# ebeauce/Seismic_BPMF

Hardware: AMD Instinct MI355X
Metric: million network-CC-samples/s (matched filter) (higher is better)
Workload: dtype f32

## Files before the change

### include/bpmf_hip.h

```cpp
#ifndef BPMF_HIP_H
#define BPMF_HIP_H

#include <stddef.h>
#include <stdint.h>

#ifdef __cplusplus
extern "C" {
#endif

typedef void *bpmf_stream_t;


const char *bpmf_last_error(void);

int bpmf_device_count(void);

int bpmf_device_info(int device, char *name, size_t name_len, size_t *total_mem_bytes,
                     int *compute_units);

#define BPMF_KERNEL_MF_MAIN 0
#define BPMF_KERNEL_BP_BEAM 1
#define BPMF_KERNEL_COUNT 2
void bpmf_profile_enable(int enable);
int bpmf_profile_count(int which_kernel);
int bpmf_profile_get_ms(int which_kernel, int launch_index, float *milliseconds);
int bpmf_profile_get_device(int which_kernel, int launch_index);

int bpmf_release_device_memory(int device);
int bpmf_device_memory_held(int device, size_t *device_bytes, size_t *pinned_bytes);
int bpmf_host_call_stats(double *out, int n);

int bpmf_set_option(const char *name, long value);
int bpmf_get_option(const char *name, long *value, long *default_value);


#define BPMF_MF_DATA_PREPARED 1
#define BPMF_MF_FORCE_DIRECT 2

size_t bpmf_mf_workspace_bytes(size_t L, size_t N, size_t T, size_t S, size_t C);

int bpmf_mf_prepare_data_dev(const float *d_data, size_t L, size_t N, size_t S, size_t C,
                             void *d_workspace, size_t workspace_bytes, bpmf_stream_t stream);

int bpmf_mf_run_dev(const float *d_templates, const int32_t *d_moveouts,
                    const float *d_weights, const float *d_data, size_t step, size_t L,
                    size_t N, size_t T, size_t S, size_t C, size_t n_corr, int network_sum,
                    int flags, void *d_workspace, size_t workspace_bytes,
                    bpmf_stream_t stream, float *d_cc_out);

#define BPMF_MF_LAUNCH_INFO_FIELDS 13
int bpmf_mf_launch_info(size_t step, size_t L, size_t N, size_t T, size_t S, size_t C, size_t n_corr,
                        int network_sum, int flags, int64_t *out);

int bpmf_mf_run(const float *templates, const int32_t *moveouts, const float *weights,
                const float *data, size_t step, size_t L, size_t N, size_t T, size_t S,
                size_t C, size_t n_corr, int network_sum, int flags, int device,
                float *cc_out);

int bpmf_mf_run_multi(const float *templates, const int32_t *moveouts, const float *weights,
                      const float *data, size_t step, size_t L, size_t N, size_t T, size_t S,
                      size_t C, size_t n_corr, int network_sum, int flags, int n_devices,
                      const int *devices, float *cc_out);

int bpmf_mf_shard_bounds(const float *weights, size_t T, size_t S, size_t C, size_t n_blocks,
                         size_t *bounds_out);

#define BPMF_BP_STRICT 0
#define BPMF_BP_FLEXIBLE 1
#define BPMF_BP_REDUCE_MAX 0
#define BPMF_BP_REDUCE_NONE 1

typedef struct bpmf_bp_plan bpmf_bp_plan;

int bpmf_bp_plan_create(const int32_t *moveouts, const float *w_sources, size_t K, size_t S,
                        size_t P, int device, int32_t source_id_offset, bpmf_bp_plan **plan);
void bpmf_bp_plan_destroy(bpmf_bp_plan *plan);

typedef struct {
    int32_t n_groups;
    int32_t tile;
    int32_t lds_bytes;
    int32_t gather_bytes;
    int32_t stations_max;
    int32_t waves_per_cu;
    int32_t n_classes;
    int32_t class_tile[3], class_sources[3], class_groups[3], class_stations_max[3];
} bpmf_bp_plan_stats;
int bpmf_bp_plan_info(const bpmf_bp_plan *plan, bpmf_bp_plan_stats *out);

size_t bpmf_bp_workspace_bytes(const bpmf_bp_plan *plan, size_t N, size_t C);

int bpmf_bp_run_dev(const bpmf_bp_plan *plan, const float *d_features,
                    const float *d_w_phases, size_t N, size_t C, int out_of_bounds,
                    int reduce, void *d_workspace, size_t workspace_bytes,
                    bpmf_stream_t stream, float *d_beam_out, int32_t *d_arg_out);

int bpmf_bp_run(const float *features, const int32_t *moveouts, const float *w_phases,
                const float *w_sources, size_t N, size_t K, size_t S, size_t C, size_t P,
                int out_of_bounds, int reduce, int device, float *beam_out, int32_t *arg_out);

int bpmf_bp_run_multi(const float *features, const int32_t *moveouts, const float *w_phases,
                      const float *w_sources, size_t N, size_t K, size_t S, size_t C, size_t P,
                      int out_of_bounds, int reduce, int n_devices, const int *devices,
// ... 142 lines not shown
```

### seismic_bpmf_amd/_lib.py

```python
import ctypes as C
import os

_HERE = os.path.dirname(os.path.abspath(__file__))
LIBPATH = os.path.join(_HERE, "lib", "libbpmf_hip.so")

_f = C.POINTER(C.c_float)
_i = C.POINTER(C.c_int32)
_u64 = C.POINTER(C.c_uint64)
_sz = C.c_size_t
_vp = C.c_void_p

class BpPlanStats(C.Structure):
    _fields_ = ([(n, C.c_int32) for n in ("n_groups", "tile", "lds_bytes", "gather_bytes",
                                          "stations_max", "waves_per_cu", "n_classes")] +
                [(n, C.c_int32 * 3) for n in ("class_tile", "class_sources", "class_groups",
                                              "class_stations_max")])


SIGNATURES = {
    "bpmf_last_error": (C.c_char_p, []),
    "bpmf_device_count": (C.c_int, []),
    "bpmf_device_info": (C.c_int, [C.c_int, C.c_char_p, _sz, C.POINTER(_sz), C.POINTER(C.c_int)]),
    "bpmf_set_option": (C.c_int, [C.c_char_p, C.c_long]),
    "bpmf_get_option": (C.c_int, [C.c_char_p, C.POINTER(C.c_long), C.POINTER(C.c_long)]),
# ... 102 lines not shown
    if rc != 0:
        msg = lib().bpmf_last_error().decode("utf-8", "replace")
        raise BpmfHipError(f"{what} failed (status {rc}): {msg}")


def last_error():
    return lib().bpmf_last_error().decode("utf-8", "replace")


def host_call_stats():
    buf = (C.c_double * 11)()
    k = lib().bpmf_host_call_stats(buf, 11)
    names = ("total_ms", "first_kernel_start_ms", "host_copy_ms", "device_wait_ms", "pieces", "fill_threads",
             "pinned_wait_ms", "copy_enqueue_ms", "plan_ms", "reserve_ms", "stragglers")
    out = {n: float(buf[i]) for i, n in enumerate(names[:k])}
    for n in ("pieces", "fill_threads", "stragglers"):
        if n in out:
            out[n] = int(out[n])
    return out


def device_count():
    n = lib().bpmf_device_count()
    if n < 0:
        check(n, "bpmf_device_count")
    return n


def device_info(device=0):
    name = C.create_string_buffer(256)
    mem = _sz(0)
    cus = C.c_int(0)
    check(lib().bpmf_device_info(device, name, 256, C.byref(mem), C.byref(cus)), "bpmf_device_info")
    return {"name": name.value.decode(), "total_mem_bytes": mem.value, "compute_units": cus.value}


KERNEL_MF_MAIN, KERNEL_BP_BEAM = 0, 1


def set_option(name, value):
    check(lib().bpmf_set_option(name.encode(), int(value)), f"bpmf_set_option({name})")


def get_option(name):
    val, dflt = C.c_long(0), C.c_long(0)
    check(lib().bpmf_get_option(name.encode(), C.byref(val), C.byref(dflt)), f"bpmf_get_option({name})")
    return val.value, dflt.value


MF_FAMILIES = ("direct", "workgroup", "wave", "split16")
MF_REFUSALS = (None, "grid too large", "more than 65535 templates on the generic kernel")


def mf_launch_info(step, L, N, T, n_stations, n_components, network_sum=True, flags=0):
    out = (C.c_int64 * 13)()
    check(lib().bpmf_mf_launch_info(step, L, N, T, n_stations, n_components, (N - L) // step + 1, 1 if network_sum else 0, int(flags), out),
          "bpmf_mf_launch_info")
    names = ("family", "maxr", "maxt", "ntile", "fused", "csplit", "sqrt_norm", "step1", "prologue", "lags_per_wg",
             "lds_bytes", "grid", "refusal")
    info = dict(zip(names, (int(x) for x in out)))
    for n in ("fused", "csplit", "sqrt_norm", "step1", "prologue"):
        info[n] = bool(info[n])
    info["family"] = MF_FAMILIES[info["family"]]
    info["refusal"] = MF_REFUSALS[info["refusal"]]
    return info


class options:

    def __init__(self, **kv):
        self.kv = {k.replace("__", "."): v for k, v in kv.items()}

    def __enter__(self):
        self.old = {k: get_option(k)[0] for k in self.kv}
        for k, v in self.kv.items():
            set_option(k, v)
        return self

    def __exit__(self, *exc):
        for k, v in self.old.items():
            set_option(k, v)
        return False


def release_device_memory(device=-1):
    check(lib().bpmf_release_device_memory(int(device)), "bpmf_release_device_memory")


def device_memory_held(device=-1):
    dv, pn = _sz(0), _sz(0)
    check(lib().bpmf_device_memory_held(int(device), C.byref(dv), C.byref(pn)), "bpmf_device_memory_held")
    return dv.value, pn.value


def profile_enable(on=True):
    lib().bpmf_profile_enable(1 if on else 0)


def _closed_launches(which):
    out = []
    for i in range(lib().bpmf_profile_count(which)):
        ms = C.c_float(0.0)
        if lib().bpmf_profile_get_ms(which, i, C.byref(ms)) == 0:
            out.append((i, ms.value))
    return out


def profile_devices(which):
    return [lib().bpmf_profile_get_device(which, i) for i, _ in _closed_launches(which)]


def profile_times_ms(which):
    return [ms for _, ms in _closed_launches(which)]


COMPAT_SWITCHES = ("mf.compat_exclusive_last_lag", "mf.compat_sqrt_norm", "mf.compat_range_all_channels",
                   "mf.compat_sequential_csum", "bp.compat_first_computed", "bp.compat_strict_upper_only",
# ... 30 lines not shown
```

### seismic_bpmf_amd/csrc/common.h

```cpp
#pragma once
#include <hip/hip_runtime.h>
#include <cstdarg>
#include <cstdint>
#include <cstdio>

namespace bpmf {

char* last_error_buf();
void set_error(const char* fmt, ...);

constexpr int CSUM_CHUNK = 1024;
constexpr float MAX_NORM = 1000.0f;

void profile_mark(int which, int edge, hipStream_t stream);

inline size_t align_up(size_t x, size_t a) { return (x + a - 1) / a * a; }

enum Option {
    OPT_BP_LDS_KB, OPT_BP_MAX_GROUP, OPT_BP_TPT, OPT_BP_REORDER, OPT_BP_DUAL,
    OPT_BP_FAST, OPT_BP_FAST_UNIFORM, OPT_BP_SPLIT, OPT_BP_VERBOSE, OPT_BP_FAST_TILE, OPT_BP_HALVES, OPT_BP_DIRECT, OPT_MF_WAVE_KERNEL, OPT_MF_MAX_MFMA_STEP, OPT_MF_HOST_BATCH_KB,
    OPT_MF_HOST_PIECE_KB, OPT_MF_VERBOSE, OPT_MF_TILES_PER_WAVE, OPT_MF_BOUNDARY_PRIO, OPT_MF_FUSED_PROLOGUE, OPT_DEBUG_POISON_OUTPUT,
    OPT_DEBUG_VIRTUAL_DEVICES, OPT_MULTI_PEER_FANOUT, OPT_MF_HOST_PIECE_LAGS, OPT_BP_HOST_PIECE_SAMPLES,
    OPT_HOST_CACHE_LIMIT_MB, OPT_BP_SLOT_PRIO, OPT_MF_CHANNEL_SPLIT, OPT_STATS_BUCKETED_MEDIAN, OPT_STATS_ROW_GRID_MIN_N, OPT_STATS_KURT_FULL_CHUNKS, OPT_MF_SPLIT16, OPT_DEBUG_FAIL_PEER_COPY,
    OPT_DEBUG_COPY_STALL_MS,
    OPT_MF_COMPAT_EXCLUSIVE_LAST_LAG, OPT_MF_COMPAT_SQRT_NORM, OPT_BP_COMPAT_FIRST_COMPUTED,
    OPT_MF_COMPAT_RANGE_ALL_CHANNELS, OPT_MF_COMPAT_SEQUENTIAL_CSUM, OPT_BP_COMPAT_STRICT_UPPER_ONLY,
    OPT_BP_COMPAT_RANGE_ALL_STATIONS, OPT_COUNT
};
long option(Option which);
unsigned long long option_generation();

hipError_t device_counts(int* n_logical, int* n_physical);
int physical_device(int logical);
extern thread_local int t_logical_device;

class DeviceGuard {
public:
    explicit DeviceGuard(int device) : DeviceGuard(device, physical_device(device)) {}
    DeviceGuard(int logical, int physical)
    {
        prev_logical_ = t_logical_device;
        t_logical_device = logical;
        err_ = hipGetDevice(&prev_);
        if (err_ == hipSuccess && prev_ != physical) {
            err_ = hipSetDevice(physical);
            switched_ = err_ == hipSuccess;
        }
    }
    ~DeviceGuard()
    {
        if (switched_) (void)hipSetDevice(prev_);
        t_logical_device = prev_logical_;
    }
    DeviceGuard(const DeviceGuard&) = delete;
    DeviceGuard& operator=(const DeviceGuard&) = delete;
    hipError_t error() const { return err_; }
private:
    int prev_ = 0, prev_logical_ = -1;
    bool switched_ = false;
    hipError_t err_ = hipSuccess;
};

}

#define BPMF_HIP_CHECK(expr)                                                          \
    do {                                                                              \
        hipError_t _e = (expr);                                                       \
        if (_e != hipSuccess) {                                                       \
            bpmf::set_error("%s failed: %s (%s:%d)", #expr, hipGetErrorString(_e),    \
                            __FILE__, __LINE__);                                      \
            return -2;                                                                \
        }                                                                             \
    } while (0)

#define BPMF_LAUNCH_CHECK() BPMF_HIP_CHECK(hipGetLastError())

#define BPMF_BIND_DEVICE(device)                 \
// ... 3 lines not shown
```

### seismic_bpmf_amd/csrc/mf.hip

```cpp
#include "common.h"
#include "context.h"
#include "mf_split_api.h"
#include <system_error>
#include <thread>
#include <chrono>
#include <vector>
#include <mutex>
#include <utility>
#include <cstring>
#include <algorithm>
#include "../../include/bpmf_hip.h"

#include <cstdlib>

namespace bpmf {

typedef float f32x16 __attribute__((ext_vector_type(16)));


__device__ __forceinline__ int2 mf_lag_range(bool any, long long mv_min, long long mv_max, long long step,
                                             long long L, long long N, long long n_corr, int exclusive_last)
{
    int2 r = make_int2(1, 0);
    if (any && N >= L) {
// ... 201 lines not shown
__device__ __forceinline__ int mf_pad(int x) { return x + (x >> 4); }

__host__ __device__ inline int mf_kpad(int L) { return (L + 15 + 15) / 16 * 16; }
__host__ __device__ inline int mf_band_len(int L) { return mf_kpad(L) + 16; }
__host__ __device__ inline int mf_window_len(int L) { return MF_LAGS_PER_WG - 16 + mf_kpad(L); }
__host__ __device__ inline int mf_buf_floats(int L)
{
    const int W = mf_window_len(L);
    return mf_band_len(L) + (W + (W >> 4) + 1);
}
__host__ inline size_t mf_lds_bytes(int L) { return ((size_t)2 * mf_buf_floats(L) + 64) * sizeof(float); }

__device__ __forceinline__ bool mf_tile_of_block(unsigned bid, int T, int n_lag_blocks, int& t,
                                                 long long& lag_block)
{
    const unsigned xcd = bid & 7u, i = bid >> 3;
    const unsigned total = (unsigned)n_lag_blocks * (unsigned)T;
    const unsigned per_xcd = (total + 7u) >> 3;
    const unsigned flat = xcd * per_xcd + i;
    t = (int)(flat % (unsigned)T);
    lag_block = (long long)(flat / (unsigned)T);
    return i < per_xcd && flat < total;
}

template <int NR, int STRIDE>
__device__ __forceinline__ void mf_stage_rows(float (&rd)[NR], __amdgpu_buffer_rsrc_t rs,
                                              long long first, int idx)
{
    const unsigned o = (unsigned)((first + idx) * 4);
    if (first >= 0) {
#pragma unroll
        for (int r = 0; r < NR; ++r)
            rd[r] = __builtin_bit_cast(float, __builtin_amdgcn_raw_buffer_load_b32(rs, (int)(o + STRIDE * 4u * r), 0, 0));
    } else {
        unsigned oo = o;
#pragma unroll
        for (int r = 0; r < NR; ++r) {
            asm volatile("" : "+v"(oo));
            rd[r] = __builtin_bit_cast(float, __builtin_amdgcn_raw_buffer_load_b32(rs, (int)oo, 0, 0));
            oo += STRIDE * 4u;
        }
    }
}
template <int NR, int STRIDE>
__device__ __forceinline__ void mf_stage_band(float (&rt)[NR], __amdgpu_buffer_rsrc_t rs, int idx)
{
    int o0 = (idx - 15) * 4;
    asm volatile("" : "+v"(o0));
    rt[0] = __builtin_bit_cast(float, __builtin_amdgcn_raw_buffer_load_b32(rs, o0, 0, 0));
#pragma unroll
    for (int r = 1; r < NR; ++r)
        rt[r] = __builtin_bit_cast(float, __builtin_amdgcn_raw_buffer_load_b32(
                                              rs, idx * 4 + (STRIDE * r - 15) * 4, 0, 0));
}

template <bool NETWORK_SUM, int MAXR, int MAXT, bool STEP1, bool SQRT_NORM = false>
__global__ __launch_bounds__(MF_THREADS, 2) void mf_mfma_kernel(
    const float* __restrict__ tmpl, const int4* __restrict__ chan_rec,
    const float* __restrict__ data, const float* __restrict__ e_d,
    const int2* __restrict__ range, int L, long long N, int T, int n_ch, long long n_corr, int step,
    float* __restrict__ out, int n_lag_blocks, int prio, int lag_block0)
{
    extern __shared__ float smem[];
    const int Kpad = mf_kpad(L);
    const int tp_len = mf_band_len(L);
    const int W = mf_window_len(L);
    const int buf_floats = mf_buf_floats(L);

    const int tid = threadIdx.x;
    const int lane = tid & 63;
    const int wv = tid >> 6;
    const int a = lane & 15;
    const int kq = lane >> 4;

    int t;
    long long lag_block;
    if (!mf_tile_of_block(blockIdx.x, T, n_lag_blocks, t, lag_block)) return;
    lag_block += lag_block0;
    const long long lag0 = lag_block * MF_LAGS_PER_WG;
    const int2 rgi = range[t];
    const int2 rg = make_int2(rgi.x * step, rgi.y * step);
    const long long nwin = N - L + 1;

    f32x4 sum[4];
#pragma unroll
    for (int u = 0; u < 4; ++u) sum[u] = (f32x4){0.0f, 0.0f, 0.0f, 0.0f};

    const bool wg_valid = rg.x <= rg.y && !(lag0 > rg.y || lag0 + MF_LAGS_PER_WG - 1 < rg.x);
    const bool wg_inside = lag0 >= rg.x && lag0 + MF_LAGS_PER_WG - 1 <= rg.y;
    const long long lag_w = lag0 + (long long)wv * MF_LAGS_PER_WAVE + 16 * a + 4 * kq;

    if (wg_valid) {
        const int a_base = 15 - a + kq;
        const int b_base = 1088 * wv + 17 * a + kq;
        const int4* __restrict__ recs = chan_rec + (size_t)t * (n_ch + 2);

        float rd[MAXR], rt[MAXT];
        auto issue_stage = [&](int ch, int mvc) {
            const __amdgpu_buffer_rsrc_t rs_d = __builtin_amdgcn_make_buffer_rsrc(
                (void*)(data + (size_t)ch * (size_t)N), 0, (int)(N * 4), 0x00020000);
            mf_stage_rows<MAXR, MF_THREADS>(rd, rs_d, lag0 + mvc, tid);
            const __amdgpu_buffer_rsrc_t rs_t = __builtin_amdgcn_make_buffer_rsrc(
                (void*)(tmpl + ((size_t)t * n_ch + ch) * (size_t)L), 0, L * 4, 0x00020000);
            mf_stage_band<MAXT, MF_THREADS>(rt, rs_t, tid);
        };
        auto write_stage = [&](float* tp, float* dw) {
// ... 455 lines not shown
                    float cc = 0.0f;
                    if (ok) {
                        cc = mf_cc_of<SQRT_NORM>(acc[u][r], et, ed[u][r]);
                        if (!NETWORK_SUM)
                            out[((size_t)t * n_corr + (STEP1 ? lag : (long long)((unsigned)lag / (unsigned)step))) * n_ch + ch] = cc;
                    }
                    if (NETWORK_SUM) sum[u][r] = __fmaf_rn(w, cc, sum[u][r]);
                }
            }
            }
            rec = rec1;
            rec1 = rec2;
            ri += REC_STRIDE;
            MF_PHASE(3);
#ifdef BPMF_PHASE_CYCLES
            ++ph_n_;
#endif
        }
    }
    if constexpr (CSPLIT) {
        __syncthreads();
        const long long lag = lag0 + tid;
        float s = 0.0f;
        if (wave_valid) {
            for (int i = 0; i < n_used; ++i) s = __fmaf_rn(__int_as_float(l_rec[i].z), exch[i * 256 + tid], s);
        }
        if (lag < n_corr) out[(size_t)t * n_corr + lag] = s;
    } else if (NETWORK_SUM) {
#pragma unroll
        for (int u = 0; u < NTILE; ++u) {
            const long long lag = lag_w + 256 * u;
            float* dst = out + (size_t)t * n_corr + lag;
            if (STEP1 && lag + 3 < n_corr) {
                *(f32x4u*)dst = sum[u];
            } else {
#pragma unroll
                for (int r = 0; r < 4; ++r) {
                    const unsigned smp = (unsigned)(lag + r);
                    const long long i = STEP1 ? (long long)smp : (long long)(smp / (unsigned)step);
                    if ((STEP1 || smp % (unsigned)step == 0) && i < n_corr) out[(size_t)t * n_corr + i] = sum[u][r];
                }
            }
        }
    }
#ifdef BPMF_PHASE_CYCLES
    if (lane == 0 && ph_n_) {
        for (int i = 0; i < 4; ++i) atomicAdd(&g_mf_phase[i], ph_acc_[i]);
        atomicAdd(&g_mf_phase[4], (unsigned long long)ph_n_);
        atomicAdd(&g_mf_phase[5], 1ull);
    }
#endif
}

template <bool NETWORK_SUM, bool SQRT_NORM = false>
__global__ __launch_bounds__(256) void mf_direct_kernel(
    const float* __restrict__ tmpl, const int* __restrict__ mv, const float* __restrict__ wgt,
    const float* __restrict__ data, const float* __restrict__ e_t,
    const float* __restrict__ e_d, const int2* __restrict__ range, long long step, int L,
    long long N, int n_ch, long long n_corr, float* __restrict__ out,
    const double* __restrict__ cs_local = nullptr, const double* __restrict__ cs_off = nullptr, long long nq = 0)
{
    const long long i = (long long)blockIdx.x * blockDim.x + threadIdx.x;
    const int t = blockIdx.y;
    if (i >= n_corr) return;
    const int2 rg = range[t];
    const bool ok = i >= rg.x && i <= rg.y;
    const long long nwin = N - L + 1;
    float sum = 0.0f;
    if (ok) {
        for (int ch = 0; ch < n_ch; ++ch) {
            const float w = wgt[(size_t)t * n_ch + ch];
            if (w == 0.0f) continue;
            const long long j = i * step + mv[(size_t)t * n_ch + ch];
            const float* tp = tmpl + ((size_t)t * n_ch + ch) * (size_t)L;
            const float* d = data + (size_t)ch * (size_t)N + j;
            float num = 0.0f;
            for (int l = 0; l < L; ++l) num = __fmaf_rn(tp[l], d[l], num);
            float cc = 0.0f;
            if constexpr (SQRT_NORM) {
                float et = 0.0f;
                for (int l = 0; l < L; ++l) et = __fmaf_rn(tp[l], tp[l], et);
                const double* lo = cs_local + (size_t)ch * (size_t)N;
                const double* of = cs_off + (size_t)ch * (size_t)nq;
                const long long nh = j + L - 1;
                const double hi = of[nh / CSUM_CHUNK] + lo[nh];
                const double low = j > 0 ? of[(j - 1) / CSUM_CHUNK] + lo[j - 1] : 0.0;
                const float den2 = et * (float)(hi - low);
                if (den2 > 1.0e-6f) cc = num / sqrtf(den2);
            } else {
                const float nrm = e_t[(size_t)t * n_ch + ch] * e_d[(size_t)ch * nwin + j];
                if (nrm < MAX_NORM) cc = num * nrm;
            }
            if (NETWORK_SUM)
                sum = __fmaf_rn(w, cc, sum);
            else
                out[((size_t)t * n_corr + i) * n_ch + ch] = cc;
        }
    }
    if (NETWORK_SUM) out[(size_t)t * n_corr + i] = sum;
}

struct MfWorkspace {
    double* local;
    double* tot;
    double* off;
    float* e_d;
// ... 37 lines not shown
                  L, T, S, C);
        return -1;
    }
    if (N < L) {
        set_error("matched filter: data (N=%zu) shorter than the templates (L=%zu)", N, L);
        return -1;
    }
    if (n_corr != (N - L) / step + 1) {
        set_error("matched filter: n_corr=%zu but (N-L)/step+1=%zu", n_corr, (N - L) / step + 1);
        return -1;
    }
    if (N > 0x7fffffffull || T * S * C > 0x7fffffffull || L > 0x7fffffffull) {
        set_error("matched filter: dimension exceeds the int32 index range");
        return -1;
    }
    return 0;
}

struct MfLaunch {
    long long off_lo = 0, off_hi = -1;
    bool first_piece = true;
};

static std::mutex g_split_days_mutex;
struct SplitDay { const void* data; size_t N, n_ch; };
static std::vector<std::pair<const void*, SplitDay>> g_split_days;
static void split_day_note(const void* ws_base, const void* data, size_t N, size_t n_ch, bool with_split)
{
    std::lock_guard<std::mutex> g(g_split_days_mutex);
    for (size_t i = 0; i < g_split_days.size(); ++i)
        if (g_split_days[i].first == ws_base) { g_split_days.erase(g_split_days.begin() + i); break; }
    if (with_split) {
        if (g_split_days.size() >= 64) g_split_days.erase(g_split_days.begin());
        g_split_days.push_back({ws_base, {data, N, n_ch}});
    }
}
static bool split_day_known(const void* ws_base, const void* data, size_t N, size_t n_ch)
{
    std::lock_guard<std::mutex> g(g_split_days_mutex);
    for (auto& e : g_split_days)
        if (e.first == ws_base) return e.second.data == data && e.second.N == N && e.second.n_ch == n_ch;
    return false;
}

enum MfFamily { MF_DIRECT = 0, MF_WORKGROUP = 1, MF_WAVE = 2, MF_SPLIT16 = 3 };
enum MfRefusal { MF_ACCEPTED = 0, MF_GRID_TOO_LARGE = 1, MF_TOO_MANY_TEMPLATES = 2 };
static const char* const MF_REFUSAL_TEXT[] = {"", "grid too large", "generic kernel supports at most 65535 templates per call"};

struct MfVariant {
    int family, refusal;
    int maxr, maxt;
    int ntile;
    bool fused, csplit;
    bool sqrt_norm, step1, prologue;
    size_t lags_wg, lds, grid;
};

constexpr int MF_WAVE_MAXT = 5;
constexpr int mf_wave_maxr(int ntile) { return ntile == 4 ? 20 : (ntile == 2 ? 12 : 8); }
static size_t mf_grid(size_t T, size_t n_blocks) { return 8 * ((T * n_blocks + 7) / 8); }

static MfVariant mf_choose(size_t step, size_t L, size_t N, size_t T, size_t n_ch, size_t n_corr, int network_sum,
                           int flags, bool ranged)
{
    MfVariant v = {};
    v.sqrt_norm = option(OPT_MF_COMPAT_SQRT_NORM) != 0;
    v.step1 = step == 1;
    v.prologue = true;
    const size_t n_offsets = (n_corr - 1) * step + 1;
    const size_t n_lag_blocks = (n_offsets + MF_LAGS_PER_WG - 1) / MF_LAGS_PER_WG;
    const int need_r = (mf_window_len((int)L) + MF_THREADS - 1) / MF_THREADS;
    const int need_t = (mf_band_len((int)L) + MF_THREADS - 1) / MF_THREADS;
    const bool mfma = step <= (size_t)option(OPT_MF_MAX_MFMA_STEP) && !(flags & BPMF_MF_FORCE_DIRECT) && need_r <= 24 &&
                      need_t <= 9 && T * (n_lag_blocks + 8) < 0x7fffffffull && N < ((size_t)1 << 30) - 8192;
    if (!mfma) {
        v.family = MF_DIRECT;
        v.lags_wg = 256;
        v.grid = (n_corr + 255) / 256 * T;
        if (T > 65535) v.refusal = MF_TOO_MANY_TEMPLATES;
        return v;
    }
    constexpr size_t SP_MIN_BLOCKS = 128;
    const size_t sp_blocks = (n_offsets + sp::LAGS_PER_WG - 1) / sp::LAGS_PER_WG;
    const bool sp_small = option(OPT_MF_SPLIT16) == 1 && T * sp_blocks < SP_MIN_BLOCKS;
    if (option(OPT_MF_SPLIT16) != 0 && sp::usable(L, N) && !sp_small) {
        v.family = MF_SPLIT16;
        v.lags_wg = sp::LAGS_PER_WG;
        v.grid = mf_grid(T, sp_blocks);
        return v;
    }
    if (option(OPT_MF_WAVE_KERNEL) == 0 || mf_kpad((int)L) > 272) {
        v.family = MF_WORKGROUP;
        v.maxr = need_r <= 20 && need_t <= 5 ? 20 : 24;
        v.maxt = v.maxr == 20 ? 5 : 9;
        v.lags_wg = MF_LAGS_PER_WG;
        v.lds = mf_lds_bytes((int)L);
        v.grid = mf_grid(T, n_lag_blocks);
        return v;
    }
    v.family = MF_WAVE;
    const size_t waves4 = T * n_lag_blocks * 4;
    v.ntile = waves4 >= 8192 ? 4 : (waves4 >= 1024 ? 2 : 1);
    const long forced = option(OPT_MF_TILES_PER_WAVE);
    if (forced == 1 || forced == 2 || forced == 4) v.ntile = (int)forced;
    v.maxr = mf_wave_maxr(v.ntile);
    v.maxt = MF_WAVE_MAXT;
    v.fused = v.ntile < 4 && n_ch <= 256 && option(OPT_MF_FUSED_PROLOGUE) != 0;
    v.prologue = !v.fused;
    const long csplit_max = option(OPT_MF_CHANNEL_SPLIT);
    v.csplit = v.ntile == 1 && v.fused && network_sum && v.step1 && n_ch <= 32 && !ranged && csplit_max > 0 &&
               waves4 * 4 <= (size_t)csplit_max;
    v.lags_wg = v.csplit ? (size_t)256 : (size_t)4 * 256 * v.ntile;
    const size_t n_blocks_w = (n_offsets + v.lags_wg - 1) / v.lags_wg;
    if (T * (n_blocks_w + 8) >= 0x7fffffffull) v.refusal = MF_GRID_TOO_LARGE;
    v.grid = mf_grid(T, n_blocks_w);
    const int Wbuf = v.ntile < 4 ? 64 * v.maxr : 256 * v.ntile - 16 + mf_kpad((int)L);
    v.lds = (size_t)4 * (mf_band_len((int)L) + (Wbuf + 2 * (Wbuf >> 4) + 2 + 63) / 64 * 64 + 64) * sizeof(float) + 256 +
            (v.fused ? 64 + (n_ch + MF_REC_TERMINATORS) * sizeof(int4) : 0) +
            (v.csplit ? n_ch * 256 * sizeof(float) : 0);
    return v;
}

}

using namespace bpmf;

extern "C" size_t bpmf_mf_workspace_bytes(size_t L, size_t N, size_t T, size_t S, size_t C)
{
    return mf_carve(nullptr, L, N, T, S * C).bytes;
}

static int mf_prepare_range(const float* d_data, size_t L, size_t N, size_t n_ch, const MfWorkspace& ws,
                            hipStream_t stream, size_t samp_lo, size_t samp_hi)
{
    const size_t nq = (N + CSUM_CHUNK - 1) / CSUM_CHUNK;
    const size_t nwin = N - L + 1;
    const size_t q_lo = samp_lo / CSUM_CHUNK, q_hi = (samp_hi + CSUM_CHUNK - 1) / CSUM_CHUNK;
    if (q_hi <= q_lo) return 0;
    {
        size_t n = n_ch * (q_hi - q_lo);
        mf_csum_local_kernel<<<dim3((unsigned)((n + 63) / 64)), dim3(64), 0, stream>>>(
            d_data, n_ch, N, nq, ws.local, ws.tot, q_lo, q_hi - q_lo);
        BPMF_LAUNCH_CHECK();
    }
    mf_csum_offsets_kernel<<<dim3((unsigned)((n_ch + 63) / 64)), dim3(64), 0, stream>>>(
        ws.tot, n_ch, nq, ws.off, q_lo, q_hi);
    BPMF_LAUNCH_CHECK();
    const size_t w_lo = samp_lo >= L - 1 ? samp_lo - (L - 1) : 0;
    const size_t w_hi = samp_hi >= N ? nwin : (samp_hi >= L - 1 ? std::min(nwin, samp_hi - (L - 1)) : 0);
    if (w_hi > w_lo) {
        mf_window_energy_kernel<<<dim3((unsigned)((w_hi - w_lo + 255) / 256), (unsigned)n_ch), dim3(256), 0,
                                  stream>>>(ws.local, ws.off, n_ch, N, nq, L, nwin,
                                            option(OPT_MF_COMPAT_SQRT_NORM) != 0 ? 1 : 0, ws.e_d, w_lo, w_hi);
        BPMF_LAUNCH_CHECK();
    }
    return 0;
}

extern "C" int bpmf_mf_prepare_data_dev(const float* d_data, size_t L, size_t N, size_t S, size_t C,
                                        void* d_workspace, size_t workspace_bytes,
                                        bpmf_stream_t stream_)
{
    hipStream_t stream = (hipStream_t)stream_;
    const size_t n_ch = S * C;
// ... 66 lines not shown
        set_error("bpmf_mf_run_dev: internal error: a range of lag blocks under mf.split16");
        return -1;
    }
    const size_t n_offsets = (n_corr - 1) * step + 1;
    const size_t off_lo = ranged ? (size_t)lc.off_lo : 0;
    const size_t off_hi = ranged ? std::min<size_t>((size_t)lc.off_hi, n_offsets) : n_offsets;
    if (off_hi <= off_lo) return 0;
    if (v.family == MF_SPLIT16 && !split_day_known(d_workspace, d_data, N, n_ch)) {
        set_error("bpmf_mf_run_dev: option mf.split16 is on but the day in this workspace was prepared without it (or is "
                  "another day): call bpmf_mf_prepare_data_dev again, or drop BPMF_MF_DATA_PREPARED");
        return -1;
    }
    if (v.refusal) {
        set_error("bpmf_mf_run_dev: %s", MF_REFUSAL_TEXT[v.refusal]);
        return -1;
    }
    const int exclusive_last = (option(OPT_MF_COMPAT_EXCLUSIVE_LAST_LAG) != 0 ? 1 : 0) |
                               (option(OPT_MF_COMPAT_RANGE_ALL_CHANNELS) != 0 ? 2 : 0);
    if (v.prologue) {
        mf_prologue_kernel<<<dim3((unsigned)T), dim3(64), 0, stream>>>(
            d_templates, d_moveouts, d_weights, (int)T, (int)n_ch, (long long)step, (long long)L, (long long)N,
            (long long)n_corr, exclusive_last, v.sqrt_norm ? 1 : 0, ws.e_t, ws.range, ws.chan_rec);
        BPMF_LAUNCH_CHECK();
    }
    if (lc.first_piece && !network_sum)
        BPMF_HIP_CHECK(hipMemsetAsync(d_cc_out, 0, T * n_corr * n_ch * sizeof(float), stream));
    else if (lc.first_piece && option(OPT_DEBUG_POISON_OUTPUT) != 0)
        BPMF_HIP_CHECK(hipMemsetAsync(d_cc_out, 0xFF, T * n_corr * sizeof(float), stream));

    const size_t nb_lo = off_lo / v.lags_wg, nb_cnt = (off_hi - off_lo + v.lags_wg - 1) / v.lags_wg;
    const dim3 grid((unsigned)mf_grid(T, nb_cnt));
    const int prio = (int)option(OPT_MF_BOUNDARY_PRIO);
    profile_mark(BPMF_KERNEL_MF_MAIN, 0, stream);
    const int rc = with_sum_step_norm(network_sum != 0, v.step1, v.sqrt_norm, [&](auto ns_c, auto s1_c, auto sq_c) -> int {
        constexpr bool NS = decltype(ns_c)::value, S1 = decltype(s1_c)::value, SQ = decltype(sq_c)::value;
        auto workgroup = [&](auto maxr_c, auto maxt_c) -> int {
            auto kern = mf_mfma_kernel<NS, decltype(maxr_c)::value, decltype(maxt_c)::value, S1, SQ>;
            if (v.lds > 64 * 1024)
                BPMF_HIP_CHECK(hipFuncSetAttribute((const void*)kern, hipFuncAttributeMaxDynamicSharedMemorySize, 160 * 1024));
            kern<<<grid, dim3(MF_THREADS), v.lds, stream>>>(
                d_templates, ws.chan_rec, d_data, ws.e_d, ws.range, (int)L, (long long)N, (int)T, (int)n_ch,
                (long long)n_corr, (int)step, d_cc_out, (int)nb_cnt, prio, (int)nb_lo);
            return 0;
        };
        auto wave = [&](auto ntile_c, auto fused_c, auto csplit_c) -> int {
            constexpr int NTILE = decltype(ntile_c)::value;
            mf_mfma_wave_kernel<NS, mf_wave_maxr(NTILE), MF_WAVE_MAXT, S1, NTILE, SQ, decltype(fused_c)::value,
                                decltype(csplit_c)::value><<<grid, dim3(MF_THREADS), v.lds, stream>>>(
                d_templates, ws.chan_rec, d_data, ws.e_d, ws.range, (int)L, (long long)N, (int)T, (int)n_ch,
                (long long)n_corr, (int)step, d_cc_out, (int)nb_cnt, prio, d_moveouts, d_weights, exclusive_last,
                (int)nb_lo);
            return 0;
        };
        auto direct = [&]() -> int {
            mf_direct_kernel<NS, SQ><<<dim3((unsigned)((n_corr + 255) / 256), (unsigned)T), dim3(256), 0, stream>>>(
                d_templates, d_moveouts, d_weights, d_data, ws.e_t, ws.e_d, ws.range, (long long)step, (int)L,
                (long long)N, (int)n_ch, (long long)n_corr, d_cc_out, ws.local, ws.off,
                (long long)((N + CSUM_CHUNK - 1) / CSUM_CHUNK));
            return 0;
        };
        const std::true_type yes{};
        const std::false_type no{};
        switch (v.family) {
            case MF_SPLIT16:
                return sp::run(d_templates, d_moveouts, ws.sp_day, ws.sp_batch, ws.chan_rec, ws.e_d, ws.range, step, L, N,
                               T, n_ch, n_corr, network_sum, v.sqrt_norm ? 1 : 0, 0, nb_cnt, d_cc_out, stream);
            case MF_WORKGROUP:
                return v.maxr == 20 ? workgroup(IntC<20>{}, IntC<5>{})
                                    : workgroup(IntC<24>{}, IntC<9>{});
            case MF_WAVE:
                if constexpr (NS && S1)
                    if (v.csplit) return wave(IntC<1>{}, yes, yes);
                if (v.ntile == 4) return wave(IntC<4>{}, no, no);
                if (v.ntile == 2) return v.fused ? wave(IntC<2>{}, yes, no) : wave(IntC<2>{}, no, no);
                return v.fused ? wave(IntC<1>{}, yes, no) : wave(IntC<1>{}, no, no);
            default:
                return direct();
        }
    });
    if (rc) return rc;
    BPMF_LAUNCH_CHECK();
    profile_mark(BPMF_KERNEL_MF_MAIN, 1, stream);
    return 0;
}

}

extern "C" int bpmf_mf_run_dev(const float* d_templates, const int32_t* d_moveouts, const float* d_weights,
                               const float* d_data, size_t step, size_t L, size_t N, size_t T, size_t S, size_t C,
                               size_t n_corr, int network_sum, int flags, void* d_workspace, size_t workspace_bytes,
                               bpmf_stream_t stream, float* d_cc_out)
{
    if (!d_templates || !d_moveouts || !d_weights || !d_data || !d_workspace || !d_cc_out) {
        set_error("bpmf_mf_run_dev: null pointer");
        return -1;
    }
    return mf_run_dev(d_templates, d_moveouts, d_weights, d_data, step, L, N, T, S, C, n_corr, network_sum, flags,
                      d_workspace, workspace_bytes, (hipStream_t)stream, d_cc_out, MfLaunch());
}

extern "C" int bpmf_mf_launch_info(size_t step, size_t L, size_t N, size_t T, size_t S, size_t C, size_t n_corr,
                                   int network_sum, int flags, int64_t* out)
{
    if (!out) {
        set_error("bpmf_mf_launch_info: null pointer");
        return -1;
    }
    if (int rc = mf_check_sizes(step, L, N, T, S, C, n_corr)) return rc;
    const MfVariant v = mf_choose(step, L, N, T, S * C, n_corr, network_sum, flags, false);
    const int64_t fields[BPMF_MF_LAUNCH_INFO_FIELDS] = {
        v.family, v.maxr, v.maxt, v.ntile, v.fused, v.csplit, v.sqrt_norm, v.step1, v.prologue,
        (int64_t)v.lags_wg, (int64_t)v.lds, (int64_t)v.grid, v.refusal};
    memcpy(out, fields, sizeof(fields));
    return 0;
}


static std::vector<size_t> mf_batch_starts(size_t T, size_t TB)
{
    std::vector<size_t> taper;
    size_t a = 2, b2 = 3, used = 0;
    while (a < TB && used + a <= T) {
        taper.push_back(a);
        used += a;
        const size_t next = b2;
        b2 = a + b2;
        a = next;
    }
    const size_t rest = T - used;
    const size_t n_full = (rest + TB - 1) / TB;
    std::vector<size_t> bt(1, 0);
    for (size_t i = 0; i < n_full; ++i)
        bt.push_back(bt.back() + rest / n_full + (i < rest % n_full ? 1 : 0));
    for (size_t i = taper.size(); i-- > 0;) bt.push_back(bt.back() + taper[i]);
    return bt;
}

static int bpmf_mf_run_impl(const float* templates, const int32_t* moveouts, const float* weights,
                           const float* data, size_t step, size_t L, size_t N, size_t T, size_t S,
                           size_t C, size_t n_corr, int network_sum, int flags, int device,
                           float* cc_out)
{
    if (!templates || !moveouts || !weights || !data || !cc_out) {
        set_error("bpmf_mf_run: null pointer");
        return -1;
    }
    if (int rc = mf_check_sizes(step, L, N, T, S, C, n_corr)) return rc;
    BPMF_BIND_DEVICE(device);
    t_call_stats = HostCallStats();
    const double t_call0 = host_now_ms();
    const size_t n_ch = S * C;
    const size_t row_bytes = n_corr * (network_sum ? 1 : n_ch) * sizeof(float);
    const long e_b = option(OPT_MF_HOST_BATCH_KB), e_p = option(OPT_MF_HOST_PIECE_KB);
    const size_t batch_bytes = e_b > 0 ? (size_t)e_b << 10 : (size_t)1 << 30;
    const size_t PIECE = e_p > 0 ? (size_t)e_p << 10 : (size_t)64 << 20;
    size_t TB = std::max<size_t>(1, batch_bytes / std::max<size_t>(row_bytes, 1));
    if (!e_b) TB = std::max<size_t>(TB, 8);
    TB = std::min(T, TB);
    const std::vector<size_t> bt = mf_batch_starts(T, TB);
    const size_t n_batch = bt.size() - 1;
    const size_t b_tp = T * n_ch * L * sizeof(float), b_mv = T * n_ch * sizeof(int32_t),
                 b_w = T * n_ch * sizeof(float), b_d = n_ch * N * sizeof(float),
                 b_out = TB * row_bytes, b_ws = bpmf_mf_workspace_bytes(L, N, TB, S, C);
    DeviceContext* ctx = device_context(device);
    if (!ctx) return -2;
// ... 180 lines not shown
```

### seismic_bpmf_amd/csrc/util.hip

```cpp
#include "common.h"
#include "../../include/bpmf_hip.h"

#include <atomic>
#include <cstring>
#include <mutex>
#include <vector>

namespace bpmf {

char* last_error_buf()
{
    static thread_local char buf[512] = {0};
    return buf;
}

void set_error(const char* fmt, ...)
{
    va_list ap;
    va_start(ap, fmt);
    vsnprintf(last_error_buf(), 512, fmt, ap);
    va_end(ap);
}

}

namespace bpmf {
namespace {
struct OptionDef { const char* name; long dflt; long lo, hi; bool plan; };
const OptionDef OPTION_DEFS[OPT_COUNT] = {
    {"bp.lds_kb", 80, 8, 160, true},
    {"bp.max_group", 4096, 1, 1 << 20, true},
    {"bp.tpt", 2, 1, 2, true},
    {"bp.reorder", 1, 0, 1, true},
    {"bp.dual", 1, 0, 1, true},
    {"bp.fast", 1, 0, 1, true},
    {"bp.fast_uniform", 1, 0, 1, true},
    {"bp.split", -1, -1, 1 << 16, false},
    {"bp.verbose", 0, 0, 1, false},
    {"bp.fast_tile", 0, 0, 512, true},
    {"bp.halves", 1, 0, 1, true},
    {"bp.direct", 0, 0, 1, true},
    {"mf.wave_kernel", 1, 0, 1, false},
    {"mf.max_mfma_step", 64, 0, 1 << 20, false},
    {"mf.host_batch_kb", 0, 0, 1L << 30, false},
    {"mf.host_piece_kb", 0, 0, 1L << 30, false},
    {"mf.verbose", 0, 0, 1, false},
    {"mf.tiles_per_wave", 0, 0, 4, false},
    {"mf.boundary_prio", 1, 0, 3, false},
    {"mf.fused_prologue", 1, 0, 1, false},
    {"debug.poison_output", 0, 0, 1, false},
    {"debug.virtual_devices", 0, 0, 64, false},
    {"multi.peer_fanout", 1, 0, 1, false},
    {"mf.host_piece_lags", 131072, 0, 1 << 24, false},
    {"bp.host_piece_samples", 131072, 0, 1 << 24, false},
    {"host.cache_limit_mb", 0, 0, 1L << 30, false},
    {"bp.slot_prio", 1, 0, 2, false},
    {"mf.channel_split", 2048, 0, 1 << 24, false},
    {"stats.bucketed_median", 2, 0, 2, false},
    {"stats.row_grid_min_n", 131072, -1, 1 << 30, false},
    {"stats.kurt_full_chunks", 1, 0, 1, false},
    {"mf.split16", 0, 0, 2, false},
    {"debug.fail_peer_copy", 0, 0, 1, false},
    {"debug.copy_stall_ms", 0, 0, 2000, false},
    {"mf.compat_exclusive_last_lag", 0, 0, 1, false},
    {"mf.compat_sqrt_norm", 0, 0, 1, false},
    {"bp.compat_first_computed", 0, 0, 1, false},
    {"mf.compat_range_all_channels", 0, 0, 1, false},
    {"mf.compat_sequential_csum", 0, 0, 1, false},
    {"bp.compat_strict_upper_only", 0, 0, 1, true},
    {"bp.compat_range_all_stations", 0, 0, 1, true},
};
std::atomic<long> g_options[OPT_COUNT];
std::once_flag g_options_once;
void init_options()
{
    for (int i = 0; i < OPT_COUNT; ++i) g_options[i].store(OPTION_DEFS[i].dflt, std::memory_order_relaxed);
}
int find_option(const char* name)
{
    if (!name) return -1;
    for (int i = 0; i < OPT_COUNT; ++i)
        if (strcmp(name, OPTION_DEFS[i].name) == 0) return i;
    return -1;
}
}

std::atomic<unsigned long long> g_option_generation{0};
unsigned long long option_generation() { return g_option_generation.load(std::memory_order_relaxed); }

long option(Option which)
{
    std::call_once(g_options_once, init_options);
    return g_options[which].load(std::memory_order_relaxed);
}

thread_local int t_logical_device = -1;

hipError_t device_counts(int* n_logical, int* n_physical)
{
    int n = 0;
    const hipError_t e = hipGetDeviceCount(&n);
    if (e != hipSuccess) n = 0;
    const long v = option(OPT_DEBUG_VIRTUAL_DEVICES);
    if (n_physical) *n_physical = n;
    if (n_logical) *n_logical = (v > 0 && n > 0) ? (int)v : n;
    return e;
}

int physical_device(int logical)
{
    if (logical < 0 || option(OPT_DEBUG_VIRTUAL_DEVICES) <= 0) return logical;
    int n = 0;
    if (hipGetDeviceCount(&n) != hipSuccess || n < 1) return logical;
    return logical % n;
}
}
// ... 185 lines not shown
```

Measured before the change: 4357.

## Add hand-scheduled chained MFMA wave kernel for 4-tile network-sum matched filter

Adds a new wave-level matched-filter kernel for the 4-tile, step-1, network-sum case with template length up to 256. It processes channels as a chain, issuing the next channel's global loads mid-way through the current one, and interleaves LDS reads with MFMA issue using explicit waitcnt and sched_barrier placement. The aim is to hide load and LDS latency and cut per-channel stalls. The new option mf.chain_tiles defaults to on, so eligible shapes route to this kernel, at the cost of heavy inline-asm scheduling that is fragile and specific to one template-padding size.

```diff
diff --git a/include/bpmf_hip.h b/include/bpmf_hip.h
--- a/include/bpmf_hip.h
+++ b/include/bpmf_hip.h
@@ -48,7 +48,7 @@
                     int flags, void *d_workspace, size_t workspace_bytes,
                     bpmf_stream_t stream, float *d_cc_out);
 
-#define BPMF_MF_LAUNCH_INFO_FIELDS 13
+#define BPMF_MF_LAUNCH_INFO_FIELDS 14
 int bpmf_mf_launch_info(size_t step, size_t L, size_t N, size_t T, size_t S, size_t C, size_t n_corr,
                         int network_sum, int flags, int64_t *out);
 
diff --git a/seismic_bpmf_amd/_lib.py b/seismic_bpmf_amd/_lib.py
--- a/seismic_bpmf_amd/_lib.py
+++ b/seismic_bpmf_amd/_lib.py
@@ -178,8 +178,8 @@
 MF_REFUSALS = (None, "grid too large", "more than 65535 templates on the generic kernel")
 
 
-def mf_launch_info(step, L, N, T, n_stations, n_components, network_sum=True, flags=0):
-    out = (C.c_int64 * 13)()
+def mf_launch_info(step, L, N, T, n_stations, n_components, network_sum=True, flags=0, detail=False):
+    out = (C.c_int64 * 14)()
     check(lib().bpmf_mf_launch_info(step, L, N, T, n_stations, n_components, (N - L) // step + 1, 1 if network_sum else 0, int(flags), out),
           "bpmf_mf_launch_info")
     names = ("family", "maxr", "maxt", "ntile", "fused", "csplit", "sqrt_norm", "step1", "prologue", "lags_per_wg",
@@ -189,6 +189,8 @@
         info[n] = bool(info[n])
     info["family"] = MF_FAMILIES[info["family"]]
     info["refusal"] = MF_REFUSALS[info["refusal"]]
+    if detail:
+        info["chain_tiles"] = int(out[13])
     return info
 
 
diff --git a/seismic_bpmf_amd/csrc/common.h b/seismic_bpmf_amd/csrc/common.h
--- a/seismic_bpmf_amd/csrc/common.h
+++ b/seismic_bpmf_amd/csrc/common.h
@@ -22,7 +22,7 @@
     OPT_MF_HOST_PIECE_KB, OPT_MF_VERBOSE, OPT_MF_TILES_PER_WAVE, OPT_MF_BOUNDARY_PRIO, OPT_MF_FUSED_PROLOGUE, OPT_DEBUG_POISON_OUTPUT,
     OPT_DEBUG_VIRTUAL_DEVICES, OPT_MULTI_PEER_FANOUT, OPT_MF_HOST_PIECE_LAGS, OPT_BP_HOST_PIECE_SAMPLES,
     OPT_HOST_CACHE_LIMIT_MB, OPT_BP_SLOT_PRIO, OPT_MF_CHANNEL_SPLIT, OPT_STATS_BUCKETED_MEDIAN, OPT_STATS_ROW_GRID_MIN_N, OPT_STATS_KURT_FULL_CHUNKS, OPT_MF_SPLIT16, OPT_DEBUG_FAIL_PEER_COPY,
-    OPT_DEBUG_COPY_STALL_MS,
+    OPT_DEBUG_COPY_STALL_MS, OPT_MF_CHAIN_TILES,
     OPT_MF_COMPAT_EXCLUSIVE_LAST_LAG, OPT_MF_COMPAT_SQRT_NORM, OPT_BP_COMPAT_FIRST_COMPUTED,
     OPT_MF_COMPAT_RANGE_ALL_CHANNELS, OPT_MF_COMPAT_SEQUENTIAL_CSUM, OPT_BP_COMPAT_STRICT_UPPER_ONLY,
     OPT_BP_COMPAT_RANGE_ALL_STATIONS, OPT_COUNT
diff --git a/seismic_bpmf_amd/csrc/mf.hip b/seismic_bpmf_amd/csrc/mf.hip
--- a/seismic_bpmf_amd/csrc/mf.hip
+++ b/seismic_bpmf_amd/csrc/mf.hip
@@ -277,6 +277,16 @@
     for (int r = 1; r < NR; ++r)
         rt[r] = __builtin_bit_cast(float, __builtin_amdgcn_raw_buffer_load_b32(
                                               rs, idx * 4 + (STRIDE * r - 15) * 4, 0, 0));
+}
+template <int NR, int STRIDE>
+__device__ __forceinline__ void mf_stage_band_periodic(float (&rt)[NR], __amdgpu_buffer_rsrc_t rs, int idx)
+{
+#pragma unroll
+    for (int r = 0; r < NR; ++r) {
+        int o = ((idx + STRIDE * r - 15) & 255) * 4;
+        asm volatile("" : "+v"(o));
+        rt[r] = __builtin_bit_cast(float, __builtin_amdgcn_raw_buffer_load_b32(rs, o, 0, 0));
+    }
 }
 
 template <bool NETWORK_SUM, int MAXR, int MAXT, bool STEP1, bool SQRT_NORM = false>
@@ -838,6 +848,258 @@
 #endif
 }
 
+template <typename F>
+__device__ __forceinline__ void mf_chain_channel(const float* tp, const float* dw, int a, int kq, int prio, float w,
+                                                 float et, const f32x4 (&ed)[4], f32x4 (&sum)[4], bool wave_inside,
+                                                 long long lag_w, int2 rg, F stage_next)
+{
+    const unsigned ab = (unsigned)(size_t)(tp + 15 - a + kq);
+    unsigned bp = (unsigned)(size_t)(dw + 18 * a + kq);
+    const unsigned cp = (unsigned)(size_t)tp;
+    const unsigned kq12 = 12u * (unsigned)kq;
+    const int zs = kq < (a & 3) ? (a >> 2) : -1;
+    f32x4 acc = (f32x4){0.0f, 0.0f, 0.0f, 0.0f}, fin = (f32x4){0.0f, 0.0f, 0.0f, 0.0f};
+    float sa[4], sb[4], d0 = 0.0f, d1 = 0.0f, d2 = 0.0f, c1 = 0.0f, c2 = 0.0f, c3 = 0.0f;
+    unsigned apq;
+#define MF_LDS_READ(dst, addr, off) \
+    asm volatile("ds_read_b32 %0, %1 offset:%2" : "=v"(dst) : "v"(addr), "n"(off))
+#define MF_MFMA(slot) acc = __builtin_amdgcn_mfma_f32_16x16x4f32(sa[slot], sb[slot], acc, 0, 0, 0)
+#define MF_STEP(cur, req, aoff, boff)                                 \
+    asm volatile("s_waitcnt lgkmcnt(2)" ::: "memory");                \
+    __builtin_amdgcn_sched_barrier(0);                                \
+    MF_MFMA(cur);                                                     \
+    __builtin_amdgcn_sched_barrier(0);                                \
+    MF_LDS_READ(sa[req], apq, (aoff));                                \
+    MF_LDS_READ(sb[req], bp, (boff));                                 \
+    __builtin_amdgcn_sched_barrier(0)
+#define MF_SLAB(g)                                                                                       \
+    {                                                                                                    \
+        const bool own = kq == (g);                                                                      \
+        const float t1 = __fmaf_rn(c1, d0, acc[1]);                                                      \
+        const float t2 = __fmaf_rn(c1, d1, __fmaf_rn(c2, d0, acc[2]));                                   \
+        const float t3 = __fmaf_rn(c1, d2, __fmaf_rn(c2, d1, __fmaf_rn(c3, d0, acc[3])));                \
+        fin[0] = own ? acc[0] : fin[0];                                                                  \
+        fin[1] = own ? t1 : fin[1];                                                                      \
+        fin[2] = own ? t2 : fin[2];                                                                      \
+        fin[3] = own ? t3 : fin[3];                                                                      \
+        acc[0] = own ? 0.0f : acc[0];                                                                    \
+        acc[1] = own ? 0.0f : acc[1];                                                                    \
+        acc[2] = own ? 0.0f : acc[2];                                                                    \
+        acc[3] = own ? 0.0f : acc[3];                                                                    \
+        sa[g] = zs == (g) ? 0.0f : sa[g];                                                                \
+    }                                                                                                    \
+    __builtin_amdgcn_sched_barrier(0)
+#define MF_CHANGE_OVER(first, last)                                   \
+    {                                                                 \
+        if (!(first)) {                                               \
+            const unsigned dp = bp + kq12;                            \
+            MF_LDS_READ(d0, dp, 0);                                   \
+            MF_LDS_READ(d1, dp, 4);                                   \
+            MF_LDS_READ(d2, dp, 8);                                   \
+            MF_LDS_READ(c1, cp, 270 * 4);                             \
+            MF_LDS_READ(c2, cp, 269 * 4);                             \
+            MF_LDS_READ(c3, cp, 268 * 4);                             \
+        }                                                             \
+        asm volatile("s_waitcnt lgkmcnt(0)" ::: "memory");            \
+        __builtin_amdgcn_sched_barrier(0);                            \
+        MF_SLAB(0);                                                   \
+        MF_MFMA(0);                                                   \
+        __builtin_amdgcn_sched_barrier(0);                            \
+        MF_LDS_READ(sa[2], ab, 1024 + 32);                            \
+        MF_LDS_READ(sb[2], bp, 32);                                   \
+        if (!(last)) {                                                \
+            MF_LDS_READ(sa[3], ab, 1024 + 48);                        \
+            MF_LDS_READ(sb[3], bp, 48);                               \
+        }                                                             \
+        __builtin_amdgcn_sched_barrier(0);                            \
+        MF_SLAB(1);                                                   \
+        MF_MFMA(1);                                                   \
+        __builtin_amdgcn_sched_barrier(0);                            \
+        if (!(last)) {                                                \
+            MF_LDS_READ(sa[0], ab, 64);                               \
+            MF_LDS_READ(sb[0], bp, 72);                               \
+            asm volatile("s_waitcnt lgkmcnt(4)" ::: "memory");        \
+        } else {                                                      \
+            asm volatile("s_waitcnt lgkmcnt(0)" ::: "memory");        \
+        }                                                             \
+        __builtin_amdgcn_sched_barrier(0);                            \
+        MF_SLAB(2);                                                   \
+        MF_MFMA(2);                                                   \
+        __builtin_amdgcn_sched_barrier(0);                            \
+        if (!(last)) {                                                \
+            MF_LDS_READ(sa[1], ab, 80);                               \
+            MF_LDS_READ(sb[1], bp, 88);                               \
+            asm volatile("s_waitcnt lgkmcnt(4)" ::: "memory");        \
+            __builtin_amdgcn_sched_barrier(0);                        \
+        }                                                             \
+        MF_SLAB(3);                                                   \
+        if (!(last)) {                                                \
+            MF_MFMA(3);                                               \
+            __builtin_amdgcn_sched_barrier(0);                        \
+        }                                                             \
+        bp += 72;                                                     \
+    }
+#define MF_PLAIN_TRIPS()                                              \
+    apq = ab + 64;                                                    \
+    _Pragma("unroll 1") for (int q = 1; q < 16; ++q) {                \
+        MF_STEP(0, 2, 32, 32);                                        \
+        MF_STEP(1, 3, 48, 48);                                        \
+        MF_STEP(2, 0, 64, 72);                                        \
+        MF_STEP(3, 1, 80, 88);                                        \
+        apq += 64;                                                    \
+        bp += 72;                                                     \
+    }
+#define MF_HAND_OVER(u)                                                                                  \
+    if (wave_inside) {                                                                                   \
+        _Pragma("unroll") for (int r = 0; r < 4; ++r)                                                    \
+            sum[u][r] = __fmaf_rn(w, mf_cc_of<false>(fin[r], et, ed[u][r]), sum[u][r]);              \
+    } else {                                                                                             \
+        _Pragma("unroll") for (int r = 0; r < 4; ++r) {                                                  \
+            const long long lag = lag_w + 256 * (u) + r;                                                 \
+            const bool ok = lag >= rg.x && lag <= rg.y;                                                  \
+            sum[u][r] = __fmaf_rn(w, ok ? mf_cc_of<false>(fin[r], et, ed[u][r]) : 0.0f, sum[u][r]);  \
+        }                                                                                                \
+    }
+    __builtin_amdgcn_sched_barrier(0);
+    if (prio) __builtin_amdgcn_s_setprio(0);
+    MF_LDS_READ(sa[0], ab, 1024);
+    MF_LDS_READ(sb[0], bp, 0);
+    MF_LDS_READ(sa[1], ab, 1024 + 16);
+    MF_LDS_READ(sb[1], bp, 16);
+    MF_CHANGE_OVER(1, 0);
+    MF_PLAIN_TRIPS();
+    MF_CHANGE_OVER(0, 0);
+    MF_HAND_OVER(0);
+    MF_PLAIN_TRIPS();
+    MF_CHANGE_OVER(0, 0);
+    MF_HAND_OVER(1);
+    stage_next();
+    __builtin_amdgcn_sched_barrier(0);
+    MF_PLAIN_TRIPS();
+    MF_CHANGE_OVER(0, 0);
+    MF_HAND_OVER(2);
+    MF_PLAIN_TRIPS();
+    MF_CHANGE_OVER(0, 1);
+    asm volatile("s_waitcnt lgkmcnt(0)" ::: "memory");
+    __builtin_amdgcn_sched_barrier(0);
+    if (prio == 1) __builtin_amdgcn_s_setprio(1);
+    else if (prio == 2) __builtin_amdgcn_s_setprio(2);
+    else if (prio == 3) __builtin_amdgcn_s_setprio(3);
+    MF_HAND_OVER(3);
+#undef MF_LDS_READ
+#undef MF_MFMA
+#undef MF_STEP
+#undef MF_SLAB
+#undef MF_CHANGE_OVER
+#undef MF_PLAIN_TRIPS
+#undef MF_HAND_OVER
+}
+
+template <int WPS>
+__global__ __launch_bounds__(MF_THREADS, WPS) void mf_mfma_wave_chain_kernel(
+    const float* __restrict__ tmpl, const int4* __restrict__ chan_rec,
+    const float* __restrict__ data, const float* __restrict__ e_d,
+    const int2* __restrict__ range, int L, long long N, int T, int n_ch, long long n_corr,
+    float* __restrict__ out, int n_lag_blocks, int prio, int lag_block0)
+{
+    extern __shared__ float smem[];
+    constexpr int MAXR = 20, MAXT = 5, LAGS_W = 1024;
+    constexpr int tp_len = 288, Ww = LAGS_W - 16 + 272;
+    constexpr int wave_floats = tp_len + (Ww + 2 * (Ww >> 4) + 2 + 63) / 64 * 64 + 64;
+    static_assert(Ww == 64 * MAXR && tp_len <= 64 * MAXT, "staging registers");
+
+    const int tid = threadIdx.x;
+    const int lane = tid & 63;
+    const int wv = __builtin_amdgcn_readfirstlane(tid >> 6);
+    const int a = lane & 15;
+    const int kq = lane >> 4;
+
+    int t;
+    long long lag_block;
+    if (!mf_tile_of_block(blockIdx.x, T, n_lag_blocks, t, lag_block)) return;
+    lag_block += lag_block0;
+    const int2 rg = range[t];
+    const long long lag0 = lag_block * (4 * LAGS_W) + (long long)wv * LAGS_W;
+    const long long nwin = N - L + 1;
+
+    f32x4 sum[4];
+#pragma unroll
+    for (int u = 0; u < 4; ++u) sum[u] = (f32x4){0.0f, 0.0f, 0.0f, 0.0f};
+
+    const bool wave_valid = rg.x <= rg.y && !(lag0 > rg.y || lag0 + LAGS_W - 1 < rg.x);
+    const bool wave_inside = lag0 >= rg.x && lag0 + LAGS_W - 1 <= rg.y;
+    const long long lag_w = lag0 + 16 * a + 4 * kq;
+
+    if (wave_valid) {
+        float* tp = smem + wv * wave_floats;
+        float* dw = tp + tp_len;
+        const int4* __restrict__ recs = chan_rec + (size_t)t * (n_ch + 2);
+        float rd[MAXR], rt[MAXT];
+        auto issue_stage = [&](int ch, int mvc) {
+            const __amdgpu_buffer_rsrc_t rs_d = __builtin_amdgcn_make_buffer_rsrc(
+                (void*)(data + (size_t)ch * (size_t)N), 0, (int)(N * 4), 0x00020000);
+            mf_stage_rows<MAXR, 64>(rd, rs_d, lag0 + mvc, lane);
+            const __amdgpu_buffer_rsrc_t rs_t = __builtin_amdgcn_make_buffer_rsrc(
+                (void*)(tmpl + ((size_t)t * n_ch + ch) * (size_t)L), 0, L * 4, 0x00020000);
+            mf_stage_band_periodic<MAXT, 64>(rt, rs_t, lane);
+        };
+        float* tpl = tp + lane;
+        float* dwl = dw + lane + 2 * (lane >> 4);
+        auto write_stage = [&]() {
+#pragma unroll
+            for (int r = 0; r < MAXT; ++r) tpl[64 * r] = rt[r];
+#pragma unroll
+            for (int r = 0; r < MAXR; ++r) dwl[72 * r] = rd[r];
+        };
+
+        int4 rec = recs[0];
+        int4 rec1 = recs[1];
+        int ri = 0;
+        if (rec.x >= 0) issue_stage(rec.x, rec.y);
+        while (rec.x >= 0) {
+            const int ch = rec.x;
+            write_stage();
+            const float w = __int_as_float(rec.z);
+            const int mvc = rec.y;
+            const float et = __int_as_float(rec.w);
+            const int4 rec2 = recs[ri + 2];
+            const float* edc = e_d + (size_t)ch * (size_t)nwin;
+            f32x4 ed[4];
+            if (wave_inside) {
+#pragma unroll
+                for (int u = 0; u < 4; ++u) ed[u] = *(const f32x4u*)(edc + lag_w + 256 * u + mvc);
+            } else {
+#pragma unroll
+                for (int u = 0; u < 4; ++u) {
+                    const long long lag = lag_w + 256 * u;
+                    if (lag + 3 >= rg.x && lag <= rg.y) {
+                        ed[u] = *(const f32x4u*)(edc + lag + mvc);
+                    } else {
+                        ed[u] = (f32x4){0.0f, 0.0f, 0.0f, 0.0f};
+                    }
+                }
+            }
+            mf_chain_channel(tp, dw, a, kq, prio, w, et, ed, sum, wave_inside, lag_w, rg,
+                             [&]() { if (rec1.x >= 0) issue_stage(rec1.x, rec1.y); });
+            rec = rec1;
+            rec1 = rec2;
+            ++ri;
+        }
+    }
+#pragma unroll
+    for (int u = 0; u < 4; ++u) {
+        const long long lag = lag_w + 256 * u;
+        float* dst = out + (size_t)t * n_corr + lag;
+        if (lag + 3 < n_corr) {
+            *(f32x4u*)dst = sum[u];
+        } else {
+#pragma unroll
+            for (int r = 0; r < 4; ++r)
+                if (lag + r < n_corr) dst[r] = sum[u][r];
+        }
+    }
+}
+
 template <bool NETWORK_SUM, bool SQRT_NORM = false>
 __global__ __launch_bounds__(256) void mf_direct_kernel(
     const float* __restrict__ tmpl, const int* __restrict__ mv, const float* __restrict__ wgt,
@@ -981,6 +1243,7 @@
     int maxr, maxt;
     int ntile;
     bool fused, csplit;
+    int chain;
     bool sqrt_norm, step1, prologue;
     size_t lags_wg, lds, grid;
 };
@@ -1039,6 +1302,8 @@
     const long csplit_max = option(OPT_MF_CHANNEL_SPLIT);
     v.csplit = v.ntile == 1 && v.fused && network_sum && v.step1 && n_ch <= 32 && !ranged && csplit_max > 0 &&
                waves4 * 4 <= (size_t)csplit_max;
+    v.chain = v.ntile == 4 && network_sum && v.step1 && !v.sqrt_norm && mf_kpad((int)L) == 272 && L <= 256
+                  ? (int)option(OPT_MF_CHAIN_TILES) : 0;
     v.lags_wg = v.csplit ? (size_t)256 : (size_t)4 * 256 * v.ntile;
     const size_t n_blocks_w = (n_offsets + v.lags_wg - 1) / v.lags_wg;
     if (T * (n_blocks_w + 8) >= 0x7fffffffull) v.refusal = MF_GRID_TOO_LARGE;
@@ -1211,6 +1476,12 @@
                 (int)nb_lo);
             return 0;
         };
+        auto wave_chain = [&](auto wps_c) -> int {
+            mf_mfma_wave_chain_kernel<decltype(wps_c)::value><<<grid, dim3(MF_THREADS), v.lds, stream>>>(
+                d_templates, ws.chan_rec, d_data, ws.e_d, ws.range, (int)L, (long long)N, (int)T, (int)n_ch,
+                (long long)n_corr, d_cc_out, (int)nb_cnt, prio, (int)nb_lo);
+            return 0;
+        };
         auto direct = [&]() -> int {
             mf_direct_kernel<NS, SQ><<<dim3((unsigned)((n_corr + 255) / 256), (unsigned)T), dim3(256), 0, stream>>>(
                 d_templates, d_moveouts, d_weights, d_data, ws.e_t, ws.e_d, ws.range, (long long)step, (int)L,
@@ -1230,6 +1501,7 @@
             case MF_WAVE:
                 if constexpr (NS && S1)
                     if (v.csplit) return wave(IntC<1>{}, yes, yes);
+                if (v.chain) return v.chain == 2 ? wave_chain(IntC<5>{}) : wave_chain(IntC<4>{});
                 if (v.ntile == 4) return wave(IntC<4>{}, no, no);
                 if (v.ntile == 2) return v.fused ? wave(IntC<2>{}, yes, no) : wave(IntC<2>{}, no, no);
                 return v.fused ? wave(IntC<1>{}, yes, no) : wave(IntC<1>{}, no, no);
@@ -1269,7 +1541,7 @@
     const MfVariant v = mf_choose(step, L, N, T, S * C, n_corr, network_sum, flags, false);
     const int64_t fields[BPMF_MF_LAUNCH_INFO_FIELDS] = {
         v.family, v.maxr, v.maxt, v.ntile, v.fused, v.csplit, v.sqrt_norm, v.step1, v.prologue,
-        (int64_t)v.lags_wg, (int64_t)v.lds, (int64_t)v.grid, v.refusal};
+        (int64_t)v.lags_wg, (int64_t)v.lds, (int64_t)v.grid, v.refusal, v.chain};
     memcpy(out, fields, sizeof(fields));
     return 0;
 }
diff --git a/seismic_bpmf_amd/csrc/util.hip b/seismic_bpmf_amd/csrc/util.hip
--- a/seismic_bpmf_amd/csrc/util.hip
+++ b/seismic_bpmf_amd/csrc/util.hip
@@ -62,6 +62,7 @@
     {"mf.split16", 0, 0, 2, false},
     {"debug.fail_peer_copy", 0, 0, 1, false},
     {"debug.copy_stall_ms", 0, 0, 2000, false},
+    {"mf.chain_tiles", 1, 0, 2, false},
     {"mf.compat_exclusive_last_lag", 0, 0, 1, false},
     {"mf.compat_sqrt_norm", 0, 0, 1, false},
     {"bp.compat_first_computed", 0, 0, 1, false},
```

New measurement: 3810. 0.874x the previous value.
